# olof3/QuantumOptimalControl.jl

Hardware: AMD Instinct MI355X
Metric: GRAPE gradient evals/sec (dim N, T slices, B seeds) @ 1/2/4/8 GPU (higher is better)
Workload: dtype f64

## Files before the change

quantumoptimalcontrol.jl_amd/csrc/qoc_blkseg.hpp:

```cpp
#pragma once
#include "qoc_blku.hpp"

namespace qoc {

struct BlksegParams {
  double rad[3];
  double mur[3], mui[3];
  double theta_cap;
  int S;
  int L;
  int UPW;
  int RB;
  const double* u;
  double* u_copy;
  double* u_copy2;
  double* J2;
  cx<double>* coef2;
  double* dJdu;
  unsigned long long* terms;
  unsigned int* done;
  double* best;
  long long seed_offset;
  double* best_res;
  double* best_out;
// ... 210 lines not shown
                                             double (&Lr)[NB * NB], double (&Li)[NB * NB], double m1r, double m1i,
                                             double m2r, double m2i, double& acc1, double& acc2) {
  constexpr int E = NB * NB;
  constexpr double invf[6] = {1.0, 1.0, 0.5, 1.0 / 6, 1.0 / 24, 1.0 / 120};
  acc1 = acc2 = 0.0;
  double Mr[MACC ? E : 1], Mi[MACC ? E : 1];
  if constexpr (MACC) {
#pragma unroll
    for (int e = 0; e < E; ++e) {
      Mr[e] = Lr[e];
      Mi[e] = Li[e];
    }
  } else {
    seg_trace<NB>(gen, Lr, Li, 1.0, m1r, m1i, m2r, m2i, acc1, acc2);
  }
  if constexpr (ORD > 1) {
    double Rr[E], Ri[E];
#pragma unroll
    for (int e = 0; e < E; ++e) {
      Rr[e] = Lr[e];
      Ri[e] = Li[e];
    }
#pragma unroll
    for (int n = 1; n < ORD; ++n) {
#pragma unroll
      for (int i = 0; i < NB; ++i) {
        double tr[NB], ti[NB];
#pragma unroll
        for (int kk = 0; kk < NB; ++kk) {
          double sr = 0.0, si = 0.0;
#pragma unroll
          for (int q = 0; q < NB; ++q) {
            sr = fma(Rr[i * NB + q], xr_[q * NB + kk], fma(-Ri[i * NB + q], xi_[q * NB + kk], sr));
            si = fma(Rr[i * NB + q], xi_[q * NB + kk], fma(Ri[i * NB + q], xr_[q * NB + kk], si));
          }
          tr[kk] = sr;
          ti[kk] = si;
        }
#pragma unroll
        for (int kk = 0; kk < NB; ++kk) {
          Rr[i * NB + kk] = tr[kk];
          Ri[i * NB + kk] = ti[kk];
        }
      }
#pragma unroll
      for (int kk = 0; kk < NB; ++kk) {
        double tr[NB], ti[NB];
#pragma unroll
        for (int i = 0; i < NB; ++i) {
          double sr = Rr[i * NB + kk], si = Ri[i * NB + kk];
#pragma unroll
          for (int q = 0; q < NB; ++q) {
            sr = fma(xr_[i * NB + q], Lr[q * NB + kk], fma(-xi_[i * NB + q], Li[q * NB + kk], sr));
            si = fma(xr_[i * NB + q], Li[q * NB + kk], fma(xi_[i * NB + q], Lr[q * NB + kk], si));
          }
          tr[i] = sr;
          ti[i] = si;
        }
#pragma unroll
        for (int i = 0; i < NB; ++i) {
          Lr[i * NB + kk] = tr[i];
          Li[i * NB + kk] = ti[i];
          if constexpr (MACC) {
            Mr[i * NB + kk] = fma(invf[n + 1], tr[i], Mr[i * NB + kk]);
            Mi[i * NB + kk] = fma(invf[n + 1], ti[i], Mi[i * NB + kk]);
          }
        }
      }
      if constexpr (!MACC) seg_trace<NB>(gen, Lr, Li, invf[n + 1], m1r, m1i, m2r, m2i, acc1, acc2);
    }
  }
  if constexpr (MACC) seg_trace<NB>(gen, Mr, Mi, 1.0, m1r, m1i, m2r, m2i, acc1, acc2);
}

struct Sk2 {
  double d0, d1, r, q;
};
__device__ __forceinline__ Sk2 sk2_of(const double2 (&e)[4]) { return Sk2{e[0].y, e[3].y, e[1].x, e[1].y}; }

template <int K = BLKSEG_KMAX>
__device__ __forceinline__ void sk2_phase(double d0, double d1, double& ct, double& st) {
  constexpr BlksegTrig T = blkseg_trig();
  const double t = 0.5 * (d0 + d1), t2 = t * t;
  ct = 0.0;
  st = 0.0;
#pragma unroll
  for (int k = K; k >= 0; --k) {
    ct = fma(ct, t2, T.c[k]);
    st = fma(st, t2, T.s[k]);
  }
  st *= t;
}
template <int K = BLKSEG_KMAX>
__device__ __forceinline__ void sk2_z(const Sk2& g0, const double* rec, double& zr, double& zi) {
  double ct, st;
  sk2_phase<K>(g0.d0, g0.d1, ct, st);
  const double2 ph = *reinterpret_cast<const double2*>(rec);
  zr = ph.x * ct - ph.y * st;
  zi = fma(ph.x, st, ph.y * ct);
}
template <int K = BLKSEG_KMAX, bool EX = false>
__device__ __forceinline__ void sk2_form(const Sk2 (&g)[3], double2 ph, double2 u, Sk2& ah, double (&ur)[4],
                                         double (&ui)[4], double* ex = nullptr) {
  constexpr BlksegTrig T = blkseg_trig();
  ah.d0 = fma(u.y, g[2].d0, fma(u.x, g[1].d0, g[0].d0));
  ah.d1 = fma(u.y, g[2].d1, fma(u.x, g[1].d1, g[0].d1));
  ah.r = fma(u.y, g[2].r, fma(u.x, g[1].r, g[0].r));
  ah.q = fma(u.y, g[2].q, fma(u.x, g[1].q, g[0].q));
  const double a = 0.5 * (ah.d0 - ah.d1);
  const double w = fma(a, a, fma(ah.r, ah.r, ah.q * ah.q));
  double cw = 0.0, sw = 0.0, s3 = 0.0, ct, st;
#pragma unroll
  for (int k = K; k >= 0; --k) {
    cw = fma(cw, w, T.c[k]);
    sw = fma(sw, w, T.s[k]);
    if constexpr (EX) s3 = fma(s3, w, T.d[k]);
  }
  sk2_phase<K>(ah.d0, ah.d1, ct, st);
  const double zr = ph.x * ct - ph.y * st, zi = fma(ph.x, st, ph.y * ct);
  const double cr = zr * cw, ci = zi * cw, sr = zr * sw, si = zi * sw;
  if constexpr (EX) {
    ex[0] = cw;
    ex[1] = sw;
    ex[2] = s3;
    ex[3] = zr;
    ex[4] = zi;
  }
  ur[0] = fma(-si, a, cr);
  ui[0] = fma(sr, a, ci);
  ur[3] = fma(si, a, cr);
  ui[3] = fma(-sr, a, ci);
  ur[1] = fma(sr, ah.r, -si * ah.q);
  ui[1] = fma(sr, ah.q, si * ah.r);
  ur[2] = fma(-sr, ah.r, -si * ah.q);
  ui[2] = fma(sr, ah.q, -si * ah.r);
}
template <int K = BLKSEG_KMAX, bool EX = false>
__device__ __forceinline__ void sk2_form_v(const Sk2 (&g)[3], double2 u, double a0, Sk2& ah, double (&v)[4],
                                           double zr = 1.0, double zi = 0.0, double* ex = nullptr) {
  constexpr BlksegTrig T = blkseg_trig();
  ah.d0 = g[0].d0;
  ah.d1 = g[0].d1;
  ah.r = fma(u.y, g[2].r, fma(u.x, g[1].r, g[0].r));
  ah.q = fma(u.y, g[2].q, fma(u.x, g[1].q, g[0].q));
  const double w = fma(a0, a0, fma(ah.r, ah.r, ah.q * ah.q));
  double cw = 0.0, sw = 0.0, s3 = 0.0;
#pragma unroll
  for (int k = K; k >= 0; --k) {
    cw = fma(cw, w, T.c[k]);
    sw = fma(sw, w, T.s[k]);
    if constexpr (EX) s3 = fma(s3, w, T.d[k]);
  }
  if constexpr (EX) {
    ex[0] = cw;
    ex[1] = sw;
    ex[2] = s3;
    ex[3] = zr;
    ex[4] = zi;
  }
  v[0] = cw;
  v[1] = sw * a0;
  v[2] = sw * ah.r;
  v[3] = sw * ah.q;
}
__device__ __forceinline__ void sk2_expand(const double (&v)[4], double (&mr)[4], double (&mi)[4]) {
  mr[0] = v[0];
  mi[0] = v[1];
  mr[1] = v[2];
  mi[1] = v[3];
  mr[2] = -v[2];
  mi[2] = v[3];
  mr[3] = v[0];
  mi[3] = -v[1];
}
__device__ __forceinline__ void sk2_vmul(const double (&v)[4], const double (&p)[4], double (&t)[4]) {
  t[0] = fma(v[0], p[0], fma(-v[1], p[1], fma(-v[2], p[2], -v[3] * p[3])));
  t[1] = fma(v[0], p[1], fma(v[1], p[0], fma(v[2], p[3], -v[3] * p[2])));
  t[2] = fma(v[0], p[2], fma(-v[1], p[3], fma(v[2], p[0], v[3] * p[1])));
  t[3] = fma(v[0], p[3], fma(v[1], p[2], fma(-v[2], p[1], v[3] * p[0])));
}

__device__ __forceinline__ void sk2_rx(double (&Rr)[4], double (&Ri)[4], const Sk2& x) {
#pragma unroll
  for (int i = 0; i < 2; ++i) {
    const double p0r = Rr[2 * i], p0i = Ri[2 * i], p1r = Rr[2 * i + 1], p1i = Ri[2 * i + 1];
    Rr[2 * i] = fma(-p0i, x.d0, fma(-p1r, x.r, -p1i * x.q));
    Ri[2 * i] = fma(p0r, x.d0, fma(p1r, x.q, -p1i * x.r));
    Rr[2 * i + 1] = fma(p0r, x.r, fma(-p0i, x.q, -p1i * x.d1));
    Ri[2 * i + 1] = fma(p0r, x.q, fma(p0i, x.r, p1r * x.d1));
  }
}
__device__ __forceinline__ void sk2_xlr(double (&Lr)[4], double (&Li)[4], const double (&Rr)[4], const double (&Ri)[4],
                                        const Sk2& x) {
#pragma unroll
  for (int k = 0; k < 2; ++k) {
    const double c0r = Lr[k], c0i = Li[k], c1r = Lr[2 + k], c1i = Li[2 + k];
    Lr[k] = fma(-x.d0, c0i, fma(x.r, c1r, fma(-x.q, c1i, Rr[k])));
    Li[k] = fma(x.d0, c0r, fma(x.r, c1i, fma(x.q, c1r, Ri[k])));
    Lr[2 + k] = fma(-x.r, c0r, fma(-x.q, c0i, fma(-x.d1, c1i, Rr[2 + k])));
    Li[2 + k] = fma(-x.r, c0i, fma(x.q, c0r, fma(x.d1, c1r, Ri[2 + k])));
  }
}
template <int ORD>
__device__ __forceinline__ void sk2_contract(const Sk2& x, const Sk2& e1, const Sk2& e2, double (&Lr)[4],
                                             double (&Li)[4], double& acc1, double& acc2) {
  constexpr double invf[6] = {1.0, 1.0, 0.5, 1.0 / 6, 1.0 / 24, 1.0 / 120};
  double Mr[4], Mi[4], Rr[4], Ri[4];
#pragma unroll
  for (int e = 0; e < 4; ++e) {
    Mr[e] = Rr[e] = Lr[e];
    Mi[e] = Ri[e] = Li[e];
  }
#pragma unroll
  for (int n = 1; n < ORD; ++n) {
    sk2_rx(Rr, Ri, x);
    sk2_xlr(Lr, Li, Rr, Ri, x);
#pragma unroll
    for (int e = 0; e < 4; ++e) {
      Mr[e] = fma(invf[n + 1], Lr[e], Mr[e]);
      Mi[e] = fma(invf[n + 1], Li[e], Mi[e]);
    }
  }
  const double dr = Mr[2] - Mr[1], di = Mi[2] + Mi[1];
  acc1 = fma(-e1.d0, Mi[0], fma(-e1.d1, Mi[3], fma(e1.r, dr, -e1.q * di)));
  acc2 = fma(-e2.d0, Mi[0], fma(-e2.d1, Mi[3], fma(e2.r, dr, -e2.q * di)));
}

template <int ORD, bool CX = false>
__device__ __forceinline__ void sk2_contract_pauli(const Sk2& x, const double (&a1)[4], const double (&a2)[4],
                                                   const double (&Kr)[4], const double (&Ki)[4], double& acc1,
                                                   double& acc2, double x0c = 0.0, double x3c = 0.0,
                                                   double x02c = 0.0) {
  static_assert(ORD >= 1 && ORD <= 3, "Pauli form for orders 1..3");
  const double k0i = Ki[0] + Ki[3], k1i = Ki[1] + Ki[2], k2i = Kr[1] - Kr[2], k3i = Ki[0] - Ki[3];
  if constexpr (CX) {
    double m1, m2;
    if constexpr (ORD == 1) {
      m1 = k1i;
      m2 = k2i;
    } else {
      const double k0r = Kr[0] + Kr[3], k1r = Kr[1] + Kr[2], k2r = Ki[2] - Ki[1];
      const double x1 = x.q, x2 = x.r;
      if constexpr (ORD == 2) {
        m1 = fma(x0c, k1r, fma(k0r, x1, k1i));
        m2 = fma(x0c, k2r, fma(k0r, x2, k2i));
      } else {
        const double di = fma(x3c, k3i, fma(x2, k2i, x1 * k1i));
        const double w = fma(x3c, x3c, fma(x2, x2, x1 * x1));
        const double al1 = fma(-0.5, x02c, fma(-1.0 / 6.0, w, 1.0));
        const double c = fma(-x0c, k0i, fma(-1.0 / 3.0, di, k0r));
        m1 = fma(al1, k1i, fma(x0c, k1r, c * x1));
        m2 = fma(al1, k2i, fma(x0c, k2r, c * x2));
      }
    }
    acc1 = -0.5 * fma(a1[2], m2, a1[1] * m1);
    acc2 = -0.5 * fma(a2[2], m2, a2[1] * m1);
    return;
  }
  double m0, m1, m2, m3;
  if constexpr (ORD == 1) {
    m0 = k0i;
    m1 = k1i;
    m2 = k2i;
    m3 = k3i;
  } else {
    const double k0r = Kr[0] + Kr[3], k1r = Kr[1] + Kr[2], k2r = Ki[2] - Ki[1], k3r = Kr[0] - Kr[3];
    const double x0 = CX ? x0c : 0.5 * (x.d0 + x.d1), x1 = x.q, x2 = x.r, x3 = CX ? x3c : 0.5 * (x.d0 - x.d1);
    const double dr = fma(x3, k3r, fma(x2, k2r, x1 * k1r)), di = fma(x3, k3i, fma(x2, k2i, x1 * k1i));
    if constexpr (ORD == 2) {
      m0 = fma(x0, k0r, k0i + dr);
      m1 = fma(x0, k1r, fma(k0r, x1, k1i));
      m2 = fma(x0, k2r, fma(k0r, x2, k2i));
      m3 = fma(x0, k3r, fma(k0r, x3, k3i));
    } else {
      const double w = fma(x3, x3, fma(x2, x2, x1 * x1)), x02 = CX ? x02c : x0 * x0;
      const double al0 = fma(-0.5, x02 + w, 1.0), al1 = fma(-0.5, x02, fma(-1.0 / 6.0, w, 1.0));
      m0 = fma(al0, k0i, fma(x0, k0r - di, dr));
      const double c = fma(-x0, k0i, fma(-1.0 / 3.0, di, k0r));
      m1 = fma(al1, k1i, fma(x0, k1r, c * x1));
      m2 = fma(al1, k2i, fma(x0, k2r, c * x2));
      m3 = fma(al1, k3i, fma(x0, k3r, c * x3));
    }
  }
  acc1 = -0.5 * fma(a1[3], m3, fma(a1[2], m2, fma(a1[1], m1, a1[0] * m0)));
  acc2 = -0.5 * fma(a2[3], m3, fma(a2[2], m2, fma(a2[1], m1, a2[0] * m0)));
}
__device__ __forceinline__ void sk2_pauli2(const Sk2& e, double (&a)[4]) {
  a[0] = e.d0 + e.d1;
  a[1] = 2.0 * e.q;
  a[2] = 2.0 * e.r;
  a[3] = e.d0 - e.d1;
}

template <bool CX = false>
__device__ __forceinline__ void sk2_contract_exact(const Sk2& x, const double (&a1)[4], const double (&a2)[4],
                                                   const double (&Kr)[4], const double (&Ki)[4], const double (&ex)[5],
                                                   double& acc1, double& acc2, double x3c = 0.0) {
  const double cw = ex[0], sw = ex[1], s3 = ex[2], zr = ex[3], zi = ex[4];
  const double k0i = Ki[0] + Ki[3], k1i = Ki[1] + Ki[2], k2i = Kr[1] - Kr[2], k3i = Ki[0] - Ki[3];
  const double k0r = Kr[0] + Kr[3], k1r = Kr[1] + Kr[2], k2r = Ki[2] - Ki[1], k3r = Kr[0] - Kr[3];
  const double x1 = x.q, x2 = x.r, x3 = CX ? x3c : 0.5 * (x.d0 - x.d1);
  const double dr = fma(x3, k3r, fma(x2, k2r, x1 * k1r)), di = fma(x3, k3i, fma(x2, k2i, x1 * k1i));
  const double cr = -fma(sw, k0i, s3 * dr), ci = fma(sw, k0r, -s3 * di);
  const double m1 = fma(zr, fma(sw, k1i, ci * x1), zi * fma(sw, k1r, cr * x1));
  const double m2 = fma(zr, fma(sw, k2i, ci * x2), zi * fma(sw, k2r, cr * x2));
  if constexpr (CX) {
    acc1 = -0.5 * fma(a1[2], m2, a1[1] * m1);
    acc2 = -0.5 * fma(a2[2], m2, a2[1] * m1);
  } else {
    const double n0r = fma(cw, k0r, -sw * di), n0i = fma(cw, k0i, sw * dr);
    const double m0 = fma(zr, n0i, zi * n0r);
    const double m3 = fma(zr, fma(sw, k3i, ci * x3), zi * fma(sw, k3r, cr * x3));
    acc1 = -0.5 * fma(a1[3], m3, fma(a1[2], m2, fma(a1[1], m1, a1[0] * m0)));
    acc2 = -0.5 * fma(a2[3], m3, fma(a2[2], m2, fma(a2[1], m1, a2[0] * m0)));
  }
}

template <int NB>
__device__ __forceinline__ void seg_rx(double (&Rr)[NB * NB], double (&Ri)[NB * NB], const double (&xr_)[NB * NB],
                                       const double (&xi_)[NB * NB]) {
#pragma unroll
  for (int i = 0; i < NB; ++i) {
    double tr[NB], ti[NB];
#pragma unroll
    for (int kk = 0; kk < NB; ++kk) {
      double sr = 0.0, si = 0.0;
#pragma unroll
      for (int q = 0; q < NB; ++q) {
        sr = fma(Rr[i * NB + q], xr_[q * NB + kk], fma(-Ri[i * NB + q], xi_[q * NB + kk], sr));
        si = fma(Rr[i * NB + q], xi_[q * NB + kk], fma(Ri[i * NB + q], xr_[q * NB + kk], si));
      }
      tr[kk] = sr;
      ti[kk] = si;
    }
#pragma unroll
    for (int kk = 0; kk < NB; ++kk) {
      Rr[i * NB + kk] = tr[kk];
      Ri[i * NB + kk] = ti[kk];
    }
  }
}
template <int NB>
__device__ __forceinline__ void seg_xlr(double (&Lr)[NB * NB], double (&Li)[NB * NB], const double (&Rr)[NB * NB],
                                        const double (&Ri)[NB * NB], const double (&xr_)[NB * NB],
                                        const double (&xi_)[NB * NB]) {
#pragma unroll
  for (int kk = 0; kk < NB; ++kk) {
    double tr[NB], ti[NB];
#pragma unroll
    for (int i = 0; i < NB; ++i) {
      double sr = Rr[i * NB + kk], si = Ri[i * NB + kk];
#pragma unroll
      for (int q = 0; q < NB; ++q) {
        sr = fma(xr_[i * NB + q], Lr[q * NB + kk], fma(-xi_[i * NB + q], Li[q * NB + kk], sr));
        si = fma(xr_[i * NB + q], Li[q * NB + kk], fma(xi_[i * NB + q], Lr[q * NB + kk], si));
      }
      tr[i] = sr;
      ti[i] = si;
    }
#pragma unroll
    for (int i = 0; i < NB; ++i) {
      Lr[i * NB + kk] = tr[i];
      Li[i * NB + kk] = ti[i];
    }
  }
}
template <int NB, typename GENF>
__device__ __forceinline__ void seg_contract_exact(GENF&& genf, const double (&xr_)[NB * NB], const double (&xi_)[NB * NB],
                                                   double (&Lr)[NB * NB], double (&Li)[NB * NB], int nex, double er,
                                                   double ei, double m1r, double m1i, double m2r, double m2i,
                                                   double& acc1, double& acc2) {
  constexpr int E = NB * NB;
  double Rr[E], Ri[E];
#pragma unroll
  for (int e = 0; e < E; ++e) {
    const double vr = Lr[e], vi = Li[e];
    Lr[e] = Rr[e] = er * vr - ei * vi;
    Li[e] = Ri[e] = fma(er, vi, ei * vr);
  }
  acc1 = acc2 = 0.0;
  seg_trace<NB>(genf(), Lr, Li, 1.0, m1r, m1i, m2r, m2i, acc1, acc2);
  double f = 1.0;
#pragma unroll 1
  for (int n = 1; n < nex; ++n) {
    seg_rx<NB>(Rr, Ri, xr_, xi_);
    seg_xlr<NB>(Lr, Li, Rr, Ri, xr_, xi_);
    f /= (double)(n + 1);
    seg_trace<NB>(genf(), Lr, Li, f, m1r, m1i, m2r, m2i, acc1, acc2);
  }
}

__device__ __forceinline__ double block_max(double v, double* scratch) {
  for (int off = 32; off > 0; off >>= 1) v = fmax(v, __shfl_xor(v, off));
  const int w = threadIdx.x >> 6, l = threadIdx.x & 63;
  __syncthreads();
  if (l == 0) scratch[w] = v;
  __syncthreads();
  double s = scratch[0];
  const int nw = (blockDim.x + 63) >> 6;
  for (int i = 1; i < nw; ++i) s = fmax(s, scratch[i]);
  __syncthreads();
  return s;
}

__device__ __forceinline__ void wave_lds_sync() {
  __builtin_amdgcn_fence(__ATOMIC_RELEASE, "wavefront");
  __builtin_amdgcn_wave_barrier();
  __builtin_amdgcn_fence(__ATOMIC_ACQUIRE, "wavefront");
}

__device__ __forceinline__ void seg_turn(int grp, int ngrp, int jj) {
  if ((grp + jj) % ngrp == 0) __builtin_amdgcn_s_setprio(1);
  else __builtin_amdgcn_s_setprio(0);
}
struct SegProg {
  int* prog;
  int partner, other;
  bool on, young;
  __device__ __forceinline__ void step(int t) {
    if (!on) return;
    if (other > t || (other == t && young)) __builtin_amdgcn_s_setprio(1);
    else __builtin_amdgcn_s_setprio(0);
    prog[threadIdx.x >> 6] = t;
    other = __builtin_amdgcn_readfirstlane(prog[partner]);
  }
};

template <int NB>
__device__ __forceinline__ void seg_pen_acc(int pm, const double (&vr)[NB * NB], const double (&vi)[NB * NB],
                                            double (&hr)[NB * NB], double (&hi)[NB * NB]) {
#pragma unroll
  for (int i = 0; i < NB; ++i)
    if ((pm >> i) & 1) {
#pragma unroll
      for (int a = 0; a < NB; ++a)
#pragma unroll
        for (int q = 0; q < NB; ++q) {
          const double ar = vr[i * NB + a], ai = vi[i * NB + a], br = vr[i * NB + q], bi = vi[i * NB + q];
          hr[a * NB + q] = fma(ar, br, fma(ai, bi, hr[a * NB + q]));
          hi[a * NB + q] = fma(ar, bi, fma(-ai, br, hi[a * NB + q]));
        }
    }
}
template <int NB, bool CF = false>
__device__ __forceinline__ void seg_pen_step(int pm, double f, double2* dp, int stride, const double (&ur)[NB * NB],
                                             const double (&ui)[NB * NB], double (&gr)[NB * NB], double (&gi)[NB * NB],
                                             double fi = 0.0) {
  double tr[NB * NB], ti[NB * NB];
#pragma unroll
  for (int e = 0; e < NB * NB; ++e) tr[e] = ti[e] = 0.0;
#pragma unroll
  for (int q = 0; q < NB; ++q) {
    double2 c[NB];
#pragma unroll
    for (int a = 0; a < NB; ++a) c[a] = dp[(a * NB + q) * stride];
    if ((pm >> q) & 1) {
#pragma unroll
      for (int a = 0; a < NB; ++a) {
        if constexpr (CF) {
          gr[a * NB + q] = fma(f, c[a].x, fma(-fi, c[a].y, gr[a * NB + q]));
          gi[a * NB + q] = fma(f, c[a].y, fma(fi, c[a].x, gi[a * NB + q]));
        } else {
          gr[a * NB + q] = fma(f, c[a].x, gr[a * NB + q]);
          gi[a * NB + q] = fma(f, c[a].y, gi[a * NB + q]);
        }
      }
    }
#pragma unroll
    for (int a = 0; a < NB; ++a)
#pragma unroll
      for (int j = 0; j < NB; ++j) {
        tr[a * NB + j] = fma(c[a].x, ur[q * NB + j], fma(-c[a].y, ui[q * NB + j], tr[a * NB + j]));
        ti[a * NB + j] = fma(c[a].x, ui[q * NB + j], fma(c[a].y, ur[q * NB + j], ti[a * NB + j]));
      }
  }
#pragma unroll
  for (int i = 0; i < NB; ++i)
#pragma unroll
    for (int j = 0; j < NB; ++j) {
      double sr = 0.0, si = 0.0;
#pragma unroll
      for (int q = 0; q < NB; ++q) {
        sr = fma(ur[q * NB + i], tr[q * NB + j], fma(ui[q * NB + i], ti[q * NB + j], sr));
        si = fma(ur[q * NB + i], ti[q * NB + j], fma(-ui[q * NB + i], tr[q * NB + j], si));
      }
      dp[(i * NB + j) * stride] = make_double2(sr, si);
    }
}

template <int NB, int ORD, int WMAX, int MODE = BLKSEG_FUSED, bool PEN = false>
__global__ __launch_bounds__(64 * WMAX) void k_blkseg_eval(const TChainArgs g, const BlkArgs bk, const BlksegParams sp) {
  extern __shared__ __attribute__((aligned(16))) unsigned char smem[];
  if constexpr (MODE == BLKSEG_BWD) {
    if (sp.stale && *sp.stale != 0) return;
  }
  constexpr int E = NB * NB;
  constexpr bool GREG = NB == 2 && WMAX <= 8;
  constexpr bool XA = NB == 2;
  constexpr int NV1 = NB == 2 ? 2 : 1;
  const int N = g.N, m = g.m, nu = g.nu, Nt = g.Nt, nblk = bk.nblk, S = sp.S, L = sp.L;
  const int tid = threadIdx.x, nthr = blockDim.x, w = tid >> 6, l = tid & 63, W = nthr >> 6;
  const int b = blockIdx.x;
  const size_t Nm = (size_t)N * m;
  BK_T(t0);
  double* const lds = reinterpret_cast<double*>(smem);
  double2* const gsh = reinterpret_cast<double2*>(lds);
  double* const rec = lds + blkseg_off_rec(NB, nblk);
// ... 65 lines not shown
  }
  auto slice = [&](int k, double2 uk) {
    const double u1 = uk.x, u2 = uk.y;
    for (int j = 0; j < nu; ++j) {
      const double v = j ? u2 : u1;
      if (sp.u_copy) sp.u_copy[((size_t)b * Nt + k) * nu + j] = v;
      if (sp.u_copy2) sp.u_copy2[((size_t)b * Nt + k) * nu + j] = v;
    }
    rmax = fmax(rmax, fma(fabs(u2), sp.rad[2], fma(fabs(u1), sp.rad[1], sp.rad[0])));
    double2* r = reinterpret_cast<double2*>(rec + 4 * (size_t)k);
    if (cmu) {
      r[0] = emu0;
    } else {
      const double mr = fma(u2, sp.mur[2], fma(u1, sp.mur[1], sp.mur[0]));
      const double mi = fma(u2, sp.mui[2], fma(u1, sp.mui[1], sp.mui[0]));
      const double er = exp(mr);
      double sn, cs;
      sincos(mi, &sn, &cs);
      r[0] = make_double2(er * cs, er * sn);
    }
    r[1] = make_double2(u1, u2);
  };
  if (tid < Nt) slice(tid, ua);
  if (tid + nthr < Nt) slice(tid + nthr, ubb);
  for (int k = tid + 2 * nthr; k < Nt; k += nthr) slice(k, load_u(k));
  rmax = block_max(rmax, red);
  int J = 0;
  double s0 = 1.0;
  while (rmax * s0 > sp.theta_cap && J < 60) {
    s0 *= 0.5;
    ++J;
  }
  int P = 0;
  {
    const double bb = rmax * s0, tol = 1.1102230246251565e-16;
    constexpr BlkuCoef K = blku_coef();
    double term = bb;
#pragma unroll
    for (int q = 0; q < BLKU_TMAX; ++q) {
      if (!(term > tol * fma(-bb, K.inv[q + 2], 1.0))) break;
      P = q + 1;
      term *= bb * K.inv[q + 2];
    }
  }
  P = __builtin_amdgcn_readfirstlane(P);
  J = __builtin_amdgcn_readfirstlane(J);
  int nex = 1;
  if constexpr (ORD == 0) nex = __builtin_amdgcn_readfirstlane(blkseg_exact_terms(rmax));
  if (tid < 8) reinterpret_cast<int*>(red + 24)[tid] = 0;
  if (J) {
    for (int k = tid; k < Nt; k += nthr) {
      rec[4 * (size_t)k + 2] *= s0;
      rec[4 * (size_t)k + 3] *= s0;
    }
  }
  __syncthreads();
  BK_T(t1);
  BK_ADD(0, t1 - t0);

  const int s = w * sp.UPW + uw;
  const bool sact = lact && s < S;
  const int kb = sact ? s * L : 0;
  const int ke = sact ? min(kb + L, Nt) : 0;
  double2 greg[GREG ? 3 : 1][GREG ? E : 1];
  if constexpr (GREG) {
#pragma unroll
    for (int j = 0; j < 3; ++j)
#pragma unroll
      for (int e = 0; e < E; ++e) greg[j][e] = gsh[(beta * 3 + j) * E + e];
  }
  auto gen_at = [&](int bc) {
    return [&, bc](int j, int e) -> double2 {
      if constexpr (GREG) return greg[j][e];
      else return gsh[(bc * 3 + j) * E + e];
    };
  };
  auto opaque = [](int v) {
    asm volatile("" : "+v"(v));
    return v;
  };

  const int grp = __builtin_amdgcn_readfirstlane(w >> 2), ngrp = (W + 3) >> 2;
  const bool turns = ngrp > 1 && SEG_TURNS && SEG_TURNMODE == 0;
  SegProg sprog;
  sprog.prog = reinterpret_cast<int*>(red + 24);
  sprog.partner = __builtin_amdgcn_readfirstlane(w ^ 4);
  sprog.on = ngrp > 1 && SEG_TURNS && SEG_TURNMODE == 1 && sprog.partner < W;
  sprog.young = grp == 1;
  sprog.other = 0;
  double qr[E], qi[E];
#pragma unroll
  for (int e = 0; e < E; ++e) {
    qr[e] = e % (NB + 1) == 0 ? 1.0 : 0.0;
    qi[e] = 0.0;
  }
  double Hr[PE], Hi[PE];
#pragma unroll
  for (int e = 0; e < PE; ++e) Hr[e] = Hi[e] = 0.0;
  const int Lf = Nt - (S - 1) * L;
  const bool fast = NB == 2 && J == 0;
  Sk2 gk[3];
  if constexpr (NB == 2) {
#pragma unroll
    for (int j = 0; j < 3; ++j) {
      double2 e4[4];
#pragma unroll
      for (int e = 0; e < 4; ++e) e4[e] = gsh[(beta * 3 + j) * E + e];
      gk[j] = sk2_of(e4);
    }
  }
  const bool zdl = NB != 2 || (gk[1].d0 == 0.0 && gk[1].d1 == 0.0 && gk[2].d0 == 0.0 && gk[2].d1 == 0.0);
  const bool zd = __syncthreads_and(zdl ? 1 : 0) != 0 && cmu && sp.mur[0] == 0.0;
  const double za0 = NB == 2 ? 0.5 * (gk[0].d0 - gk[0].d1) : 0.0;
  const int ksel = __builtin_amdgcn_readfirstlane(blkseg_series_k(rmax * s0));
  const bool su = fast && zd;
  double pq[4] = {1.0, 0.0, 0.0, 0.0};
  auto lane_z = [&](double& zr, double& zi) {
    zr = 1.0;
    zi = 0.0;
    if constexpr (NB == 2) {
      if (su) {
        if (ksel == 5) sk2_z<5>(gk[0], rec, zr, zi);
        else if (ksel == 7) sk2_z<7>(gk[0], rec, zr, zi);
        else sk2_z<BLKSEG_KMAX>(gk[0], rec, zr, zi);
      }
    }
  };
  auto p1_fast = [&](int jj, auto SEL_, auto K_, auto ZD_) {
    constexpr bool SEL = decltype(SEL_)::value;
    constexpr int KS = decltype(K_)::value;
    constexpr bool ZD = decltype(ZD_)::value;
    if constexpr (NB == 2) {
    if constexpr (ZD) {
      double vv[2][4];
      bool act[2];
#pragma unroll
      for (int v = 0; v < 2; ++v) {
        const int k = kb + jj + v;
        act[v] = !SEL || (sact && jj + v < L && k < ke);
        const double* r = rec + 4 * (size_t)(act[v] ? k : 0);
        Sk2 ah;
        sk2_form_v<KS>(gk, *reinterpret_cast<const double2*>(r + 2), za0, ah, vv[v]);
      }
#pragma unroll
      for (int v = 0; v < 2; ++v) {
        double t[4];
        sk2_vmul(vv[v], pq, t);
#pragma unroll
        for (int e = 0; e < 4; ++e) pq[e] = !SEL || act[v] ? t[e] : pq[e];
        if constexpr (PEN) {
          if (pm && (!SEL || act[v])) {
            double wr_[4], wi_[4];
            sk2_expand(pq, wr_, wi_);
            seg_pen_acc<NB>(pm, wr_, wi_, Hr, Hi);
          }
        }
      }
    } else {
      double ur[2][4], ui[2][4];
      bool act[2];
#pragma unroll
      for (int v = 0; v < 2; ++v) {
        const int k = kb + jj + v;
        act[v] = !SEL || (sact && jj + v < L && k < ke);
        const double* r = rec + 4 * (size_t)(act[v] ? k : 0);
        Sk2 ah;
        sk2_form<KS>(gk, *reinterpret_cast<const double2*>(r), *reinterpret_cast<const double2*>(r + 2), ah, ur[v],
                     ui[v]);
      }
#pragma unroll
      for (int v = 0; v < 2; ++v) {
        double tr[4], ti[4];
        seg_mm<2, false, false>(ur[v], ui[v], qr, qi, tr, ti);
#pragma unroll
        for (int e = 0; e < 4; ++e) {
          qr[e] = !SEL || act[v] ? tr[e] : qr[e];
          qi[e] = !SEL || act[v] ? ti[e] : qi[e];
        }
        if constexpr (PEN) {
          if (pm && (!SEL || act[v])) seg_pen_acc<NB>(pm, qr, qi, Hr, Hi);
        }
      }
    }
    }
  };
  auto loop1z = [&](auto K_, auto ZD_) {
    for (int jj = 0; jj < L; jj += 2) {
      if (turns) seg_turn(grp, ngrp, jj >> 1);
      sprog.step(jj >> 1);
      if (jj + 1 < Lf) p1_fast(jj, std::false_type(), K_, ZD_);
      else p1_fast(jj, std::true_type(), K_, ZD_);
    }
    if constexpr (NB == 2) {
      if constexpr (decltype(ZD_)::value) sk2_expand(pq, qr, qi);
    }
  };
  auto loop1 = [&](auto K_) {
    if (zd) loop1z(K_, std::true_type());
    else loop1z(K_, std::false_type());
  };
  double Gr[E], Gi[E];
  auto gseg_at = [&](int e) -> double2& { return sp.gseg[(((size_t)b * E + e) * S + s) * nblk + beta]; };
  auto dl_at = [&](int e) -> double2& { return slot[((size_t)s * E + e) * nblk + beta]; };
  auto dseg_at = [&](int e) -> double2& { return sp.dseg[(((size_t)b * E + e) * S + s) * nblk + beta]; };
  if constexpr (MODE == BLKSEG_BWD) {
#pragma unroll
    for (int e = 0; e < E; ++e) {
      const double2 v = sact ? gseg_at(e) : make_double2(0.0, 0.0);
      Gr[e] = v.x;
      Gi[e] = v.y;
    }
    if constexpr (PEN) {
      if (pm)
#pragma unroll
        for (int e = 0; e < E; ++e) dl_at(e) = dseg_at(e);
    }
    if (sp.coef2 && tid < 2 * m) sp.coef2[(size_t)b * 2 * m + tid] = g.coef[(size_t)b * 2 * m + tid];
  } else {
  if (fast) {
    if (ksel == 5) loop1(std::integral_constant<int, 5>());
    else if (ksel == 7) loop1(std::integral_constant<int, 7>());
    else loop1(std::integral_constant<int, BLKSEG_KMAX>());
  } else {
    for (int jj = 0; jj < L; jj += NV1) {
      if (turns) seg_turn(grp, ngrp, jj / NV1);
      sprog.step(jj / NV1);
      const double* rk[NV1];
      bool act[NV1];
#pragma unroll
      for (int v = 0; v < NV1; ++v) {
        const int k = kb + jj + v;
        act[v] = sact && jj + v < L && k < ke;
        rk[v] = rec + 4 * (size_t)(act[v] ? k : 0);
      }
      double ar[NV1][E], ai[NV1][E], ur[NV1][E], ui[NV1][E];
      seg_form<NB, NV1>(gen_at(GREG ? beta : opaque(beta)), rk, s0, P, J, ar, ai, ur, ui);
#pragma unroll
      for (int v = 0; v < NV1; ++v) {
        double tr[E], ti[E];
        seg_mm<NB, false, false>(ur[v], ui[v], qr, qi, tr, ti);
#pragma unroll
        for (int e = 0; e < E; ++e) {
          qr[e] = act[v] ? tr[e] : qr[e];
          qi[e] = act[v] ? ti[e] : qi[e];
        }
        if constexpr (PEN) {
          if (pm && act[v]) seg_pen_acc<NB>(pm, qr, qi, Hr, Hi);
        }
      }
    }
  }
  if constexpr (PEN) {
    if (pm) {
      double tr[E], ti[E];
      seg_mm<NB, false, false>(qr, qi, Hr, Hi, tr, ti);
      seg_mm<NB, false, true>(tr, ti, qr, qi, Hr, Hi);
    }
    if (w == 0 && l < nblk) {
      double dr[E], di[E];
#pragma unroll
      for (int e = 0; e < E; ++e) dr[e] = di[e] = 0.0;
      if (pm)
        for (int c = 0; c < m; ++c) {
          if (!((sp.pcol >> c) & 1u)) continue;
          double xr[NB], xi[NB];
#pragma unroll
          for (int i = 0; i < NB; ++i) {
            const size_t o = 2 * ((size_t)c * N + max(brw[i], 0));
            xr[i] = brw[i] >= 0 ? xN[o] : 0.0;
            xi[i] = brw[i] >= 0 ? xN[o + 1] : 0.0;
          }
#pragma unroll
          for (int a = 0; a < NB; ++a)
#pragma unroll
// ... 319 lines not shown
          }
        __builtin_amdgcn_sched_barrier(0);
        const double f = 2.0 * sp.pen_mu;
#pragma unroll
        for (int i = 0; i < NB; ++i)
#pragma unroll
          for (int j = 0; j < NB; ++j) {
            double sr = 0.0, si = 0.0;
#pragma unroll
            for (int q = 0; q < NB; ++q) {
              sr = fma(dr[i * NB + q], Hr[q * NB + j], fma(-di[i * NB + q], Hi[q * NB + j], sr));
              si = fma(dr[i * NB + q], Hi[q * NB + j], fma(di[i * NB + q], Hr[q * NB + j], si));
            }
            hr[i * NB + j] = fma(f, sr, hr[i * NB + j]);
            hi[i * NB + j] = fma(f, si, hi[i * NB + j]);
          }
        __builtin_amdgcn_sched_barrier(0);
      }
    }
    seg_mm<NB, false, false>(qr, qi, hr, hi, tr, ti);
    seg_mm<NB, false, true>(tr, ti, qr, qi, Gr, Gi);
  }

  if (!early) publish();
  BK_T(t2e);
  BK_ADD(2, t2e - t2);
  if constexpr (MODE == BLKSEG_FWD) {
    if (sact)
#pragma unroll
      for (int e = 0; e < E; ++e) gseg_at(e) = make_double2(Gr[e], Gi[e]);
    if (sp.terms && tid == 0) atomicAdd(sp.terms + b % TERM_SLOTS, (unsigned long long)Nt * ((unsigned long long)P << J));
    return;
  }
  }
  BK_T(t3);
  const double mu1r = sp.mur[1], mu1i = sp.mui[1], mu2r = sp.mur[2], mu2i = sp.mui[2];
  const double pen2 = PEN ? 2.0 * sp.pen_mu : 0.0;
  auto pen_step = [&](const double (&ur)[E], const double (&ui)[E]) {
    seg_pen_step<NB>(pm, pen2, slot + (size_t)opaque(s) * E * nblk + beta, nblk, ur, ui, Gr, Gi);
  };
  double zr, zi;
  lane_z(zr, zi);
  if (su) {
#pragma unroll
    for (int e = 0; e < E; ++e) {
      const double t = fma(zr, Gr[e], zi * Gi[e]);
      Gi[e] = fma(zr, Gi[e], -zi * Gr[e]);
      Gr[e] = t;
    }
  }
  const double pen2r = pen2 * zr, pen2i = -pen2 * zi;
  auto pen_step_v = [&](const double (&ur)[E], const double (&ui)[E]) {
    seg_pen_step<NB, true>(pm, pen2r, slot + (size_t)opaque(s) * E * nblk + beta, nblk, ur, ui, Gr, Gi, pen2i);
  };
  double* const wr = wred + 128 * RB * w;
  const int nrl = sp.UPW * max(nu, 1);
  const int rq = l / nrl, rrem = l - rq * nrl, ro = rrem / max(nu, 1), rj = rrem - ro * max(nu, 1);
  int rslot = 0;
  auto reduce = [&](int jj, double acc1, double acc2) {
    const int r = rslot;
    rslot = r == RB - 1 ? 0 : r + 1;
    *reinterpret_cast<double2*>(wr + 128 * r + 2 * l) = make_double2(acc1, acc2);
    if (r == RB - 1 || jj == 0) {
      wave_lds_sync();
      if (rq <= r) {
        const int ss = w * sp.UPW + ro, kk = ss * L + jj + r - rq;
        if (ss < S && kk < Nt) {
          const double* src = wr + 128 * rq + 2 * ro * nblk + rj;
          double sum = 0.0;
          for (int q = 0; q < nblk; ++q) sum += src[2 * q];
          dJ[(size_t)kk * nu + rj] = sum;
        }
      }
      wave_lds_sync();
    }
  };
  double pa1[4] = {0, 0, 0, 0}, pa2[4] = {0, 0, 0, 0};
  const double zxd0 = NB == 2 ? gk[0].d0 + sp.mui[0] : 0.0, zxd1 = NB == 2 ? gk[0].d1 + sp.mui[0] : 0.0;
  const double zx0 = 0.5 * (zxd0 + zxd1), zx3 = 0.5 * (zxd0 - zxd1), zx02 = zx0 * zx0;
  if constexpr (NB == 2) {
    sk2_pauli2(Sk2{gk[1].d0 + mu1i, gk[1].d1 + mu1i, gk[1].r, gk[1].q}, pa1);
    sk2_pauli2(Sk2{gk[2].d0 + mu2i, gk[2].d1 + mu2i, gk[2].r, gk[2].q}, pa2);
  }
  auto p3_fast = [&](int jj, auto SEL_, auto K_, auto ZD_) {
    constexpr bool SEL = decltype(SEL_)::value;
    constexpr int KS = decltype(K_)::value;
    constexpr bool ZD = decltype(ZD_)::value;
    if constexpr (NB == 2) {
      const int k = kb + jj;
      const bool act = !SEL || (sact && k < ke);
      const double* r = rec + 4 * (size_t)(act ? k : 0);
      const double2 u = *reinterpret_cast<const double2*>(r + 2);
      Sk2 ah;
      double ur[4], ui[4], ex[5];
      if constexpr (ZD) {
        double vv[4];
        sk2_form_v<KS, ORD == 0>(gk, u, za0, ah, vv, zr, zi, ex);
        sk2_expand(vv, ur, ui);
      } else {
        sk2_form<KS, ORD == 0>(gk, *reinterpret_cast<const double2*>(r), u, ah, ur, ui, ex);
      }
      if constexpr (PEN) {
        if (pm && (!SEL || act)) {
          if constexpr (ZD) pen_step_v(ur, ui);
          else pen_step(ur, ui);
        }
      }
      double Kr[4], Ki[4], tr[4], ti[4];
      seg_mm<2, true, false>(ur, ui, Gr, Gi, Kr, Ki);
      seg_mm<2, false, false>(Kr, Ki, ur, ui, tr, ti);
#pragma unroll
      for (int e = 0; e < 4; ++e) {
        Gr[e] = !SEL || act ? tr[e] : Gr[e];
        Gi[e] = !SEL || act ? ti[e] : Gi[e];
      }
      const double mki = ZD ? sp.mui[0] : fma(u.y, mu2i, fma(u.x, mu1i, sp.mui[0]));
      const Sk2 x{ah.d0 + mki, ah.d1 + mki, ah.r, ah.q};
      double acc1, acc2;
      if constexpr (ORD == 0) {
        sk2_contract_exact<ZD>(x, pa1, pa2, Kr, Ki, ex, acc1, acc2, zx3);
      } else if constexpr (ORD <= 3) {
        sk2_contract_pauli<ORD, ZD>(x, pa1, pa2, Kr, Ki, acc1, acc2, zx0, zx3, zx02);
      } else {
        const Sk2 e1{gk[1].d0 + mu1i, gk[1].d1 + mu1i, gk[1].r, gk[1].q};
        const Sk2 e2{gk[2].d0 + mu2i, gk[2].d1 + mu2i, gk[2].r, gk[2].q};
        sk2_contract<ORD>(x, e1, e2, Kr, Ki, acc1, acc2);
      }
      reduce(jj, !SEL || act ? acc1 : 0.0, !SEL || act ? acc2 : 0.0);
    }
  };
  auto loop3z = [&](auto K_, auto ZD_) {
    for (int jj = L - 1; jj >= 0; --jj) {
      if (turns) seg_turn(grp, ngrp, jj);
      sprog.step(L + (L - 1 - jj));
      if (jj < Lf) p3_fast(jj, std::false_type(), K_, ZD_);
      else p3_fast(jj, std::true_type(), K_, ZD_);
    }
  };
  auto loop3 = [&](auto K_) {
    if (zd) loop3z(K_, std::true_type());
    else loop3z(K_, std::false_type());
  };
  if (fast) {
    if (ksel == 5) loop3(std::integral_constant<int, 5>());
    else if (ksel == 7) loop3(std::integral_constant<int, 7>());
    else loop3(std::integral_constant<int, BLKSEG_KMAX>());
  } else {
    for (int jj = L - 1; jj >= 0; --jj) {
      if (turns) seg_turn(grp, ngrp, jj);
      sprog.step(L + (L - 1 - jj));
      const int k = kb + jj;
      const bool act = sact && k < ke;
      const double* rk[1] = {rec + 4 * (size_t)(act ? k : 0)};
      const auto gen = gen_at(GREG ? beta : opaque(beta));
      double ar[1][E], ai[1][E], ur[1][E], ui[1][E];
      seg_form<NB, 1>(gen, rk, s0, P, J, ar, ai, ur, ui);
      if constexpr (PEN) {
        if (pm && act) pen_step(ur[0], ui[0]);
      }
      double Kr[E], Ki[E], tr[E], ti[E];
      seg_mm<NB, true, false>(ur[0], ui[0], Gr, Gi, Kr, Ki);
      seg_mm<NB, false, false>(Kr, Ki, ur[0], ui[0], tr, ti);
#pragma unroll
      for (int e = 0; e < E; ++e) {
        Gr[e] = act ? tr[e] : Gr[e];
        Gi[e] = act ? ti[e] : Gi[e];
      }
      const double2 su = *reinterpret_cast<const double2*>(rk[0] + 2);
      const double u1 = ldexp(su.x, J), u2 = ldexp(su.y, J);
      const double mkr = fma(u2, sp.mur[2], fma(u1, sp.mur[1], sp.mur[0]));
      const double mki = fma(u2, sp.mui[2], fma(u1, sp.mui[1], sp.mui[0]));
      const double dgr = ORD == 0 ? 0.0 : mkr, dgi = ORD == 0 ? 0.0 : mki;
      double xr[E], xi[E];
      if constexpr (XA) {
#pragma unroll
        for (int e = 0; e < E; ++e) {
          xr[e] = (J ? ldexp(ar[0][e], J) : ar[0][e]) + (e % (NB + 1) == 0 ? dgr : 0.0);
          xi[e] = (J ? ldexp(ai[0][e], J) : ai[0][e]) + (e % (NB + 1) == 0 ? dgi : 0.0);
        }
      } else {
        const auto gen2 = gen_at(opaque(beta));
#pragma unroll
        for (int e = 0; e < E; ++e) {
          const double2 g0 = gen2(0, e), g1 = gen2(1, e), g2 = gen2(2, e);
          xr[e] = fma(u2, g2.x, fma(u1, g1.x, g0.x)) + (e % (NB + 1) == 0 ? dgr : 0.0);
          xi[e] = fma(u2, g2.y, fma(u1, g1.y, g0.y)) + (e % (NB + 1) == 0 ? dgi : 0.0);
        }
      }
      double acc1, acc2;
      constexpr bool GST = ORD == 0 && NB == 3 && !PEN;
      if constexpr (GST) {
        double2* const gp = slot + (size_t)opaque(sact ? s : 0) * E * nblk + beta;
        if (sact)
#pragma unroll
          for (int e = 0; e < E; ++e) gp[e * nblk] = make_double2(Gr[e], Gi[e]);
      }
      if constexpr (ORD == 0) {
        seg_contract_exact<NB>([&] { return gen_at(GREG ? beta : opaque(beta)); }, xr, xi, Kr, Ki, nex, rk[0][0],
                               rk[0][1], mu1r, mu1i, mu2r, mu2i, acc1, acc2);
      } else {
        seg_contract<NB, ORD, XA>(gen, xr, xi, Kr, Ki, mu1r, mu1i, mu2r, mu2i, acc1, acc2);
      }
      if constexpr (GST) {
        const double2* const gp = slot + (size_t)opaque(sact ? s : 0) * E * nblk + beta;
#pragma unroll
        for (int e = 0; e < E; ++e) {
          const double2 v = gp[e * nblk];
          Gr[e] = v.x;
          Gi[e] = v.y;
        }
      }
      reduce(jj, act ? acc1 : 0.0, act ? acc2 : 0.0);
    }
  }
  if (turns || sprog.on) __builtin_amdgcn_s_setprio(0);
  BK_T(t4);
  BK_ADD(3, t4 - t3);
  SEGW_SET(16 + w, t4 - t0);
  __syncthreads();
// ... 11 lines not shown
```

Before: 4.199 million.

## Peel polynomial loops, fold scaling into Pauli coefs, prefetch controls, split loops

Starts the Horner trig evaluations at the top coefficient, which drops one fma per series. Folds the -0.5 scale into the precomputed Pauli coefficients so it is no longer applied per step. Splits the forward and backward segment loops into unselected and selected parts so the hot path has no per-iteration branch. In the backward zero-drift path it prefetches the next step's control values with a sched barrier, and it defers the readfirstlane on the partner-progress read to hide LDS latency. These are several small independent tweaks, with some extra register pressure from the prefetch.

```diff
diff --git a/quantumoptimalcontrol.jl_amd/csrc/qoc_blkseg.hpp b/quantumoptimalcontrol.jl_amd/csrc/qoc_blkseg.hpp
--- a/quantumoptimalcontrol.jl_amd/csrc/qoc_blkseg.hpp
+++ b/quantumoptimalcontrol.jl_amd/csrc/qoc_blkseg.hpp
@@ -316,10 +316,10 @@
 __device__ __forceinline__ void sk2_phase(double d0, double d1, double& ct, double& st) {
   constexpr BlksegTrig T = blkseg_trig();
   const double t = 0.5 * (d0 + d1), t2 = t * t;
-  ct = 0.0;
-  st = 0.0;
-#pragma unroll
-  for (int k = K; k >= 0; --k) {
+  ct = T.c[K];
+  st = T.s[K];
+#pragma unroll
+  for (int k = K - 1; k >= 0; --k) {
     ct = fma(ct, t2, T.c[k]);
     st = fma(st, t2, T.s[k]);
   }
@@ -343,9 +343,9 @@
   ah.q = fma(u.y, g[2].q, fma(u.x, g[1].q, g[0].q));
   const double a = 0.5 * (ah.d0 - ah.d1);
   const double w = fma(a, a, fma(ah.r, ah.r, ah.q * ah.q));
-  double cw = 0.0, sw = 0.0, s3 = 0.0, ct, st;
-#pragma unroll
-  for (int k = K; k >= 0; --k) {
+  double cw = T.c[K], sw = T.s[K], s3 = EX ? T.d[K] : 0.0, ct, st;
+#pragma unroll
+  for (int k = K - 1; k >= 0; --k) {
     cw = fma(cw, w, T.c[k]);
     sw = fma(sw, w, T.s[k]);
     if constexpr (EX) s3 = fma(s3, w, T.d[k]);
@@ -378,9 +378,9 @@
   ah.r = fma(u.y, g[2].r, fma(u.x, g[1].r, g[0].r));
   ah.q = fma(u.y, g[2].q, fma(u.x, g[1].q, g[0].q));
   const double w = fma(a0, a0, fma(ah.r, ah.r, ah.q * ah.q));
-  double cw = 0.0, sw = 0.0, s3 = 0.0;
-#pragma unroll
-  for (int k = K; k >= 0; --k) {
+  double cw = T.c[K], sw = T.s[K], s3 = EX ? T.d[K] : 0.0;
+#pragma unroll
+  for (int k = K - 1; k >= 0; --k) {
     cw = fma(cw, w, T.c[k]);
     sw = fma(sw, w, T.s[k]);
     if constexpr (EX) s3 = fma(s3, w, T.d[k]);
@@ -487,8 +487,8 @@
         m2 = fma(al1, k2i, fma(x0c, k2r, c * x2));
       }
     }
-    acc1 = -0.5 * fma(a1[2], m2, a1[1] * m1);
-    acc2 = -0.5 * fma(a2[2], m2, a2[1] * m1);
+    acc1 = fma(a1[2], m2, a1[1] * m1);
+    acc2 = fma(a2[2], m2, a2[1] * m1);
     return;
   }
   double m0, m1, m2, m3;
@@ -516,14 +516,14 @@
       m3 = fma(al1, k3i, fma(x0, k3r, c * x3));
     }
   }
-  acc1 = -0.5 * fma(a1[3], m3, fma(a1[2], m2, fma(a1[1], m1, a1[0] * m0)));
-  acc2 = -0.5 * fma(a2[3], m3, fma(a2[2], m2, fma(a2[1], m1, a2[0] * m0)));
+  acc1 = fma(a1[3], m3, fma(a1[2], m2, fma(a1[1], m1, a1[0] * m0)));
+  acc2 = fma(a2[3], m3, fma(a2[2], m2, fma(a2[1], m1, a2[0] * m0)));
 }
 __device__ __forceinline__ void sk2_pauli2(const Sk2& e, double (&a)[4]) {
-  a[0] = e.d0 + e.d1;
-  a[1] = 2.0 * e.q;
-  a[2] = 2.0 * e.r;
-  a[3] = e.d0 - e.d1;
+  a[0] = -0.5 * (e.d0 + e.d1);
+  a[1] = -0.5 * (2.0 * e.q);
+  a[2] = -0.5 * (2.0 * e.r);
+  a[3] = -0.5 * (e.d0 - e.d1);
 }
 
 template <bool CX = false>
@@ -539,14 +539,14 @@
   const double m1 = fma(zr, fma(sw, k1i, ci * x1), zi * fma(sw, k1r, cr * x1));
   const double m2 = fma(zr, fma(sw, k2i, ci * x2), zi * fma(sw, k2r, cr * x2));
   if constexpr (CX) {
-    acc1 = -0.5 * fma(a1[2], m2, a1[1] * m1);
-    acc2 = -0.5 * fma(a2[2], m2, a2[1] * m1);
+    acc1 = fma(a1[2], m2, a1[1] * m1);
+    acc2 = fma(a2[2], m2, a2[1] * m1);
   } else {
     const double n0r = fma(cw, k0r, -sw * di), n0i = fma(cw, k0i, sw * dr);
     const double m0 = fma(zr, n0i, zi * n0r);
     const double m3 = fma(zr, fma(sw, k3i, ci * x3), zi * fma(sw, k3r, cr * x3));
-    acc1 = -0.5 * fma(a1[3], m3, fma(a1[2], m2, fma(a1[1], m1, a1[0] * m0)));
-    acc2 = -0.5 * fma(a2[3], m3, fma(a2[2], m2, fma(a2[1], m1, a2[0] * m0)));
+    acc1 = fma(a1[3], m3, fma(a1[2], m2, fma(a1[1], m1, a1[0] * m0)));
+    acc2 = fma(a2[3], m3, fma(a2[2], m2, fma(a2[1], m1, a2[0] * m0)));
   }
 }
 
@@ -647,16 +647,18 @@
   if ((grp + jj) % ngrp == 0) __builtin_amdgcn_s_setprio(1);
   else __builtin_amdgcn_s_setprio(0);
 }
+template <bool DEFER>
 struct SegProg {
   int* prog;
   int partner, other;
   bool on, young;
   __device__ __forceinline__ void step(int t) {
     if (!on) return;
-    if (other > t || (other == t && young)) __builtin_amdgcn_s_setprio(1);
+    const int o = DEFER ? __builtin_amdgcn_readfirstlane(other) : other;
+    if (o > t || (o == t && young)) __builtin_amdgcn_s_setprio(1);
     else __builtin_amdgcn_s_setprio(0);
     prog[threadIdx.x >> 6] = t;
-    other = __builtin_amdgcn_readfirstlane(prog[partner]);
+    other = DEFER ? prog[partner] : __builtin_amdgcn_readfirstlane(prog[partner]);
   }
 };
 
@@ -888,7 +890,7 @@
 
   const int grp = __builtin_amdgcn_readfirstlane(w >> 2), ngrp = (W + 3) >> 2;
   const bool turns = ngrp > 1 && SEG_TURNS && SEG_TURNMODE == 0;
-  SegProg sprog;
+  SegProg<NB == 2 && MODE != BLKSEG_FWD> sprog;
   sprog.prog = reinterpret_cast<int*>(red + 24);
   sprog.partner = __builtin_amdgcn_readfirstlane(w ^ 4);
   sprog.on = ngrp > 1 && SEG_TURNS && SEG_TURNMODE == 1 && sprog.partner < W;
@@ -932,6 +934,7 @@
       }
     }
   };
+  const double* const reck = rec + 4 * (size_t)kb;
   auto p1_fast = [&](int jj, auto SEL_, auto K_, auto ZD_) {
     constexpr bool SEL = decltype(SEL_)::value;
     constexpr int KS = decltype(K_)::value;
@@ -944,7 +947,7 @@
       for (int v = 0; v < 2; ++v) {
         const int k = kb + jj + v;
         act[v] = !SEL || (sact && jj + v < L && k < ke);
-        const double* r = rec + 4 * (size_t)(act[v] ? k : 0);
+        const double* r = SEL ? rec + 4 * (size_t)(act[v] ? k : 0) : reck + 4 * (size_t)(jj + v);
         Sk2 ah;
         sk2_form_v<KS>(gk, *reinterpret_cast<const double2*>(r + 2), za0, ah, vv[v]);
       }
@@ -969,7 +972,7 @@
       for (int v = 0; v < 2; ++v) {
         const int k = kb + jj + v;
         act[v] = !SEL || (sact && jj + v < L && k < ke);
-        const double* r = rec + 4 * (size_t)(act[v] ? k : 0);
+        const double* r = SEL ? rec + 4 * (size_t)(act[v] ? k : 0) : reck + 4 * (size_t)(jj + v);
         Sk2 ah;
         sk2_form<KS>(gk, *reinterpret_cast<const double2*>(r), *reinterpret_cast<const double2*>(r + 2), ah, ur[v],
                      ui[v]);
@@ -991,11 +994,16 @@
     }
   };
   auto loop1z = [&](auto K_, auto ZD_) {
-    for (int jj = 0; jj < L; jj += 2) {
+    int jj = 0;
+    for (; jj + 1 < Lf; jj += 2) {
       if (turns) seg_turn(grp, ngrp, jj >> 1);
       sprog.step(jj >> 1);
-      if (jj + 1 < Lf) p1_fast(jj, std::false_type(), K_, ZD_);
-      else p1_fast(jj, std::true_type(), K_, ZD_);
+      p1_fast(jj, std::false_type(), K_, ZD_);
+    }
+    for (; jj < L; jj += 2) {
+      if (turns) seg_turn(grp, ngrp, jj >> 1);
+      sprog.step(jj >> 1);
+      p1_fast(jj, std::true_type(), K_, ZD_);
     }
     if constexpr (NB == 2) {
       if constexpr (decltype(ZD_)::value) sk2_expand(pq, qr, qi);
@@ -1481,15 +1489,15 @@
     sk2_pauli2(Sk2{gk[1].d0 + mu1i, gk[1].d1 + mu1i, gk[1].r, gk[1].q}, pa1);
     sk2_pauli2(Sk2{gk[2].d0 + mu2i, gk[2].d1 + mu2i, gk[2].r, gk[2].q}, pa2);
   }
-  auto p3_fast = [&](int jj, auto SEL_, auto K_, auto ZD_) {
+  auto p3_fast = [&](int jj, auto SEL_, auto K_, auto ZD_, const double2* upre = nullptr) {
     constexpr bool SEL = decltype(SEL_)::value;
     constexpr int KS = decltype(K_)::value;
     constexpr bool ZD = decltype(ZD_)::value;
     if constexpr (NB == 2) {
       const int k = kb + jj;
       const bool act = !SEL || (sact && k < ke);
-      const double* r = rec + 4 * (size_t)(act ? k : 0);
-      const double2 u = *reinterpret_cast<const double2*>(r + 2);
+      const double* r = SEL ? rec + 4 * (size_t)(act ? k : 0) : reck + 4 * (size_t)jj;
+      const double2 u = upre ? *upre : *reinterpret_cast<const double2*>(r + 2);
       Sk2 ah;
       double ur[4], ui[4], ex[5];
       if constexpr (ZD) {
@@ -1529,11 +1537,24 @@
     }
   };
   auto loop3z = [&](auto K_, auto ZD_) {
-    for (int jj = L - 1; jj >= 0; --jj) {
+    int jj = L - 1;
+    for (; jj >= Lf; --jj) {
       if (turns) seg_turn(grp, ngrp, jj);
       sprog.step(L + (L - 1 - jj));
-      if (jj < Lf) p3_fast(jj, std::false_type(), K_, ZD_);
-      else p3_fast(jj, std::true_type(), K_, ZD_);
+      p3_fast(jj, std::true_type(), K_, ZD_);
+    }
+    constexpr bool PRE = decltype(ZD_)::value;
+    double2 un = make_double2(0.0, 0.0);
+    if (PRE && jj >= 0) un = *reinterpret_cast<const double2*>(reck + 4 * (size_t)jj + 2);
+    for (; jj >= 0; --jj) {
+      if (turns) seg_turn(grp, ngrp, jj);
+      sprog.step(L + (L - 1 - jj));
+      const double2 uc = un;
+      if constexpr (PRE) {
+        un = *reinterpret_cast<const double2*>(reck + 4 * (size_t)max(jj - 1, 0) + 2);
+        __builtin_amdgcn_sched_barrier(0);
+      }
+      p3_fast(jj, std::false_type(), K_, ZD_, PRE ? &uc : nullptr);
     }
   };
   auto loop3 = [&](auto K_) {
```

Result: faster. 4.757 million, median of 6 (+13.3%).
